# svip-lab/impersonator

Hardware: AMD Instinct MI355X
Metric: frames/sec (256x256 motion-imitation, batch=8) (higher is better)
Workload: dtype bf16x3; 1 GPU; Imitator inference 256x256 batch=8, random-init ImpersonatorGenerator + synthetic SMPL, 1 source; frames=1024, batch_per_gpu=8, image_size=256, parallelism=frame-sharded replicas x1, grid_sample_align_corners=False, lanes=2, batches_per_launch_sequence=4, frames_per_launch=32, precision=bf16x3, precision_policy=auto

## Files before the change

### impersonator_amd/csrc/heads.hip

```cpp
#include <type_traits>

#include "conv.h"

namespace lwg {
namespace {

typedef float f32x16 __attribute__((ext_vector_type(16)));
typedef __bf16 bf16x8_t __attribute__((ext_vector_type(8)));

constexpr int HS_COLS = 32;
constexpr int HS_OUT = HS_COLS - 6;
constexpr int HS_KS = 4;
constexpr int HS_NF = 7 * HS_KS;
constexpr int HS_UP = 33;

__global__ __launch_bounds__(256) void heads_pack_kernel(const float *__restrict__ wh, uint4 *__restrict__ wfrag)
{
    const int i = blockIdx.x * blockDim.x + threadIdx.x;
    if (i >= HS_NF * 2 * 64) return;
    const int lane = i & 63, plane = (i >> 6) & 1, f = i >> 7;
    const int kh = f / HS_KS, ks = f - kh * HS_KS;
    const int n = lane & 31, k8 = (lane >> 5) * 8;
    const int kw = n >> 2, o = n & 3;
    bf16x8_t out;
#pragma unroll
    for (int e = 0; e < 8; ++e) {
        const int c = ks * 16 + k8 + e;
        const float v = n < 28 ? wh[((size_t)(kh * 7 + kw) * 64 + c) * 4 + o] : 0.f;
        const __bf16 hi = (__bf16)v;
        out[e] = plane == 0 ? hi : (__bf16)(v - (float)hi);
    }
    wfrag[i] = __builtin_bit_cast(uint4, out);
}

struct HeadsGeom {
    int strips, bands, band_rows;
};

struct RowRegs {
    float4 raw[2 * HS_KS];
};

__global__ __launch_bounds__(64) void heads_bf16x3_kernel(const HeadsArgs a, const uint4 *__restrict__ wfrag,
                                                          const HeadsGeom g)
{
    __shared__ float2 s_ss[64];
    __shared__ float s_u[HS_COLS * HS_UP];
    __shared__ uint4 s_bl[HS_NF * 64];
    const int lane = threadIdx.x;
    const int strip = blockIdx.x % g.strips;
    const int band = (blockIdx.x / g.strips) % g.bands;
    const int n = blockIdx.x / (g.strips * g.bands);
    const int xs0 = strip * HS_OUT;
    const int y0 = band * g.band_rows;
    const int y1 = min(y0 + g.band_rows, a.H);
    if (y0 >= y1) return;

    s_ss[lane] = a.scale_shift[(size_t)n * 64 + lane];
    bf16x8_t bh[HS_NF];
#pragma unroll
    for (int f = 0; f < HS_NF; ++f) {
        bh[f] = __builtin_bit_cast(bf16x8_t, wfrag[(f * 2 + 0) * 64 + lane]);
        s_bl[f * 64 + lane] = wfrag[(f * 2 + 1) * 64 + lane];
    }
    __syncthreads();

    const int m = lane & 31, kh2 = lane >> 5;
    const int xp = xs0 - 3 + m;
    const bool col_ok = xp >= 0 && xp < a.W;
    const float *xin = a.x + ((size_t)n * a.H * a.W + (col_ok ? xp : 0)) * 64 + kh2 * 8;
    const size_t row_stride = (size_t)a.W * 64;

    constexpr int RING = 8;
    f32x16 acc[RING];
#pragma unroll
    for (int s = 0; s < RING; ++s)
#pragma unroll
        for (int r = 0; r < 16; ++r) acc[s][r] = 0.f;

    struct Frag { bf16x8_t hi[HS_KS], lo[HS_KS]; };
    RowRegs raw[2];
    Frag frag;
    auto load_row = [&](int r, RowRegs &dst) {
        const int rc = min(max(r, 0), a.H - 1);
        const float *p = xin + (size_t)rc * row_stride;
#pragma unroll
        for (int ks = 0; ks < HS_KS; ++ks) {
            dst.raw[2 * ks] = *reinterpret_cast<const float4 *>(p + ks * 16);
            dst.raw[2 * ks + 1] = *reinterpret_cast<const float4 *>(p + ks * 16 + 4);
        }
    };
    auto convert = [&](int r, const RowRegs &src, int ks, Frag &f) {
        const bool ok = col_ok && r >= 0 && r < a.H;
        const float4 q0 = src.raw[2 * ks], q1 = src.raw[2 * ks + 1];
        const float raw8[8] = {q0.x, q0.y, q0.z, q0.w, q1.x, q1.y, q1.z, q1.w};
        const float4 *ssp = reinterpret_cast<const float4 *>(s_ss + ks * 16 + kh2 * 8);
        bf16x8_t h, l;
#pragma unroll
        for (int e2 = 0; e2 < 4; ++e2) {
            const float4 ss2 = ssp[e2];
            const float v0 = fmaxf(fmaf(raw8[2 * e2], ss2.x, ss2.y), 0.f);
            const float v1 = fmaxf(fmaf(raw8[2 * e2 + 1], ss2.z, ss2.w), 0.f);
            const __bf16 h0 = (__bf16)v0, h1 = (__bf16)v1;
            h[2 * e2] = h0;
            h[2 * e2 + 1] = h1;
            l[2 * e2] = (__bf16)(v0 - (float)h0);
            l[2 * e2 + 1] = (__bf16)(v1 - (float)h1);
        }
        const uint4 hz = __builtin_bit_cast(uint4, h), lz = __builtin_bit_cast(uint4, l);
        f.hi[ks] = __builtin_bit_cast(bf16x8_t, ok ? hz : make_uint4(0u, 0u, 0u, 0u));
        f.lo[ks] = __builtin_bit_cast(bf16x8_t, ok ? lz : make_uint4(0u, 0u, 0u, 0u));
    };

    const size_t hw = (size_t)a.H * a.W;
    const int xl = lane & 31, half = lane >> 5;
    const int oxc = min(xs0 + min(xl, HS_OUT - 1), a.W - 1);
    const float *bgp = a.pred ? a.bg + (size_t)(a.bg_bs > 1 ? n : 0) * 3 * hw : a.x;
    struct Bg { float v[2]; };
    auto load_bg = [&](int y) {
        const size_t p = (size_t)min(max(y, 0), a.H - 1) * a.W + oxc;
        Bg b;
        b.v[0] = bgp[(size_t)(half * 2) * hw + p];
        b.v[1] = bgp[(size_t)(half ? 2 : 1) * hw + p];
        return b;
    };
    struct Out { float c0, c1, msk; };
    auto tile_to_lds = [&](const f32x16 &u) {
        const int col = lane & 31, rsel = 4 * (lane >> 5);
#pragma unroll
        for (int r = 0; r < 16; ++r) s_u[((r & 3) + 8 * (r >> 2) + rsel) * HS_UP + col] = u[r];
    };
    auto reduce_row = [&]() {
        const int xr = min(xl, HS_OUT - 1);
        float s0 = 0.f, s1 = 0.f;
#pragma unroll
        for (int kw = 0; kw < 7; ++kw) {
            s0 += s_u[(xr + kw) * HS_UP + kw * 4 + half * 2];
            s1 += s_u[(xr + kw) * HS_UP + kw * 4 + half * 2 + 1];
        }
        const float e0 = __expf(2.f * s0);
        const float e1 = __expf(half ? -s1 : 2.f * s1);
        const float r0 = __builtin_amdgcn_rcpf(1.f + e0), r1 = __builtin_amdgcn_rcpf(1.f + e1);
        Out o;
        o.c0 = fmaf(-2.f, r0, 1.f);
        o.c1 = half ? r1 : fmaf(-2.f, r1, 1.f);
        o.msk = __shfl(o.c1, 32 + xl);
        return o;
    };
    auto store_row = [&](const Out &o, const Bg &b, int y) {
        const int ox = xs0 + xl;
        if (y < y0 || y >= y1 || xl >= HS_OUT || ox >= a.W) return;
        const size_t p = (size_t)y * a.W + ox;
        const float cv[2] = {o.c0, o.c1};
#pragma unroll
        for (int k = 0; k < 2; ++k) {
            const int c = half * 2 + k;
            if (c == 3) {
                if (a.mask) a.mask[(size_t)n * hw + p] = o.msk;
                continue;
            }
            if (a.color) a.color[((size_t)n * 3 + c) * hw + p] = cv[k];
            if (a.pred) a.pred[((size_t)n * 3 + c) * hw + p] = o.msk * b.v[k] + (1.f - o.msk) * cv[k];
        }
    };

    const int niter = y1 - y0 + 6;
    load_row(y0 - 3, raw[0]);
    load_row(y0 - 2, raw[1]);
#pragma unroll
    for (int ks = 0; ks < HS_KS; ++ks) convert(y0 - 3, raw[0], ks, frag);

    auto row_step = [&](int it, auto ph_c) {
        constexpr int PH = decltype(ph_c)::value;
        constexpr int PREV = (PH + RING - 1) % RING;
        const int r = y0 - 3 + it;
        const Bg bgv = load_bg(r - 4);
        load_row(r + 2, raw[PH & 1]);
        tile_to_lds(acc[PREV]);
#pragma unroll
        for (int q = 0; q < 16; ++q) acc[PREV][q] = 0.f;
        Out o;
#pragma unroll
        for (int ks = 0; ks < HS_KS; ++ks) {
            bf16x8_t bl[7];
#pragma unroll
            for (int kh = 0; kh < 7; ++kh) bl[kh] = __builtin_bit_cast(bf16x8_t, s_bl[(kh * HS_KS + ks) * 64 + lane]);
#pragma unroll
            for (int t = 0; t < 3; ++t)
#pragma unroll
                for (int kh = 0; kh < 7; ++kh) {
                    const int slot = (PH - kh + 6 + RING) % RING;
                    const bf16x8_t av = t == 0 ? frag.lo[ks] : frag.hi[ks];
                    const bf16x8_t bv = t == 2 ? bl[kh] : bh[kh * HS_KS + ks];
                    acc[slot] = __builtin_amdgcn_mfma_f32_32x32x16_bf16(av, bv, acc[slot], 0, 0, 0);
                }
            if (ks == 1) o = reduce_row();
            convert(r + 1, raw[(PH + 1) & 1], ks, frag);
#pragma unroll
            for (int g2 = 0; g2 < 21; ++g2) {
                __builtin_amdgcn_sched_group_barrier(0x008, 1, 0);
                __builtin_amdgcn_sched_group_barrier(0x002, 6, 0);
                __builtin_amdgcn_sched_group_barrier(0x100, 1, 0);
            }
            __builtin_amdgcn_sched_barrier(0);
        }
        store_row(o, bgv, r - 4);
    };

    for (int it = 0; it < niter; it += RING) {
        row_step(it, std::integral_constant<int, 0>{});
        if (it + 1 < niter) row_step(it + 1, std::integral_constant<int, 1>{});
        if (it + 2 < niter) row_step(it + 2, std::integral_constant<int, 2>{});
        if (it + 3 < niter) row_step(it + 3, std::integral_constant<int, 3>{});
        if (it + 4 < niter) row_step(it + 4, std::integral_constant<int, 4>{});
        if (it + 5 < niter) row_step(it + 5, std::integral_constant<int, 5>{});
        if (it + 6 < niter) row_step(it + 6, std::integral_constant<int, 6>{});
        if (it + 7 < niter) row_step(it + 7, std::integral_constant<int, 7>{});
    }
    {
        const int last = niter - 1, y = y0 - 3 + last - 3;
        const Bg bgv = load_bg(y);
        switch (last % RING) {
            case 0: tile_to_lds(acc[0]); break;
            case 1: tile_to_lds(acc[1]); break;
            case 2: tile_to_lds(acc[2]); break;
            case 3: tile_to_lds(acc[3]); break;
            case 4: tile_to_lds(acc[4]); break;
            case 5: tile_to_lds(acc[5]); break;
            case 6: tile_to_lds(acc[6]); break;
            default: tile_to_lds(acc[7]); break;
        }
        const Out o = reduce_row();
        store_row(o, bgv, y);
    }
}

}

size_t heads_bf16x3_frag_bytes() { return (size_t)HS_NF * 2 * 64 * 16; }

int launch_heads_pack(const float *wh, void *wfrag, hipStream_t st)
{
    heads_pack_kernel<<<ceil_div(HS_NF * 2 * 64, 256), 256, 0, st>>>(wh, static_cast<uint4 *>(wfrag));
    LWG_LAUNCH_CHECK("heads_pack_kernel");
    return LWG_OK;
}

int launch_heads_bf16x3(const HeadsArgs &a, const void *wfrag, hipStream_t st, int bands_forced)
{
    if (a.pred && !a.bg) LWG_FAIL(LWG_ERR_INVALID_ARG, "heads: pred requested without a background image");
    if (!wfrag) LWG_FAIL(LWG_ERR_STATE, "heads: packed weight fragments missing");
    if (a.N < 1 || a.H < 1 || a.W < 1 || bands_forced < 0) LWG_FAIL(LWG_ERR_INVALID_ARG, "heads: empty tensor or negative band count");
    HeadsGeom g;
    g.strips = ceil_div(a.W, HS_OUT);
    const int target = 4 * device_cu_count();
    int bands = target / (g.strips * a.N);
    if (bands < 1) bands = 1;
    if (bands > ceil_div(a.H, 8)) bands = ceil_div(a.H, 8);
    if (bands_forced > 0) bands = bands_forced < a.H ? bands_forced : a.H;
    g.band_rows = ceil_div(a.H, bands);
    g.bands = ceil_div(a.H, g.band_rows);
    heads_bf16x3_kernel<<<g.strips * g.bands * a.N, 64, 0, st>>>(a, static_cast<const uint4 *>(wfrag), g);
    LWG_LAUNCH_CHECK("heads_bf16x3_kernel");
    return LWG_OK;
}

}
```

Measured before the change: 3931 frames/s.

## Hand-interleave heads conv MFMA loop with loads, conversion, reduction; add trace probe

Restructures the heads kernel's inner row step so each of the 21 MFMAs per k-slice is paired with a slice of other work: LDS weight loads, split bf16 hi/lo conversion, staged tile-to-LDS writes, reduction reads and activation, all fenced with scheduling barriers and register pins. The aim is to hide LDS latency and VALU work behind the matrix instructions instead of relying on the sched_group_barrier hints. It also adds an optional timing-trace variant behind a compile flag and an environment variable. The manual schedule increases register pressure and makes the code fragile.

```diff
diff --git a/impersonator_amd/csrc/heads.hip b/impersonator_amd/csrc/heads.hip
--- a/impersonator_amd/csrc/heads.hip
+++ b/impersonator_amd/csrc/heads.hip
@@ -1,3 +1,5 @@
+#include <cstdio>
+#include <cstdlib>
 #include <type_traits>
 
 #include "conv.h"
@@ -7,6 +9,9 @@
 
 typedef float f32x16 __attribute__((ext_vector_type(16)));
 typedef __bf16 bf16x8_t __attribute__((ext_vector_type(8)));
+typedef __bf16 bf16x2_t __attribute__((ext_vector_type(2)));
+typedef unsigned u32x4 __attribute__((ext_vector_type(4)));
+typedef float f32x4 __attribute__((ext_vector_type(4)));
 
 constexpr int HS_COLS = 32;
 constexpr int HS_OUT = HS_COLS - 6;
@@ -41,9 +46,29 @@
     float4 raw[2 * HS_KS];
 };
 
-__global__ __launch_bounds__(64) void heads_bf16x3_kernel(const HeadsArgs a, const uint4 *__restrict__ wfrag,
-                                                          const HeadsGeom g)
-{
+template <bool TRACE>
+__device__ __forceinline__ void heads_bf16x3_body(const HeadsArgs &a, const uint4 *__restrict__ wfrag, const HeadsGeom &g,
+                                                  unsigned long long *__restrict__ trace)
+{
+    auto stamp = [&]() -> unsigned long long {
+        if constexpr (TRACE) {
+            __builtin_amdgcn_sched_barrier(0);
+            const unsigned long long t = __builtin_amdgcn_s_memtime();
+            __builtin_amdgcn_sched_barrier(0);
+            return t;
+        }
+        return 0ull;
+    };
+    unsigned long long tr_vm = 0, tr_lgkm = 0, tr_cal = 0, tr_ks[HS_KS] = {0, 0, 0, 0}, tr_store = 0;
+    const unsigned long long tr_in = stamp();
+    unsigned long long tr_rt0 = 0;
+    if constexpr (TRACE) {
+        tr_rt0 = __builtin_amdgcn_s_memrealtime();
+        const unsigned long long c0 = stamp();
+        asm volatile("s_waitcnt lgkmcnt(0)" ::: "memory");
+        const unsigned long long c1 = stamp();
+        tr_cal = c1 - c0;
+    }
     __shared__ float2 s_ss[64];
     __shared__ float s_u[HS_COLS * HS_UP];
     __shared__ uint4 s_bl[HS_NF * 64];
@@ -55,6 +80,7 @@
     const int y0 = band * g.band_rows;
     const int y1 = min(y0 + g.band_rows, a.H);
     if (y0 >= y1) return;
+    const int tr_stores = (a.color ? 2 : 0) + (a.mask ? 1 : 0) + (a.pred ? 2 : 0);
 
     s_ss[lane] = a.scale_shift[(size_t)n * 64 + lane];
     bf16x8_t bh[HS_NF];
@@ -81,14 +107,15 @@
     struct Frag { bf16x8_t hi[HS_KS], lo[HS_KS]; };
     RowRegs raw[2];
     Frag frag;
-    auto load_row = [&](int r, RowRegs &dst) {
+    auto load_row_part = [&](int r, RowRegs &dst, int ks) {
         const int rc = min(max(r, 0), a.H - 1);
         const float *p = xin + (size_t)rc * row_stride;
-#pragma unroll
-        for (int ks = 0; ks < HS_KS; ++ks) {
-            dst.raw[2 * ks] = *reinterpret_cast<const float4 *>(p + ks * 16);
-            dst.raw[2 * ks + 1] = *reinterpret_cast<const float4 *>(p + ks * 16 + 4);
-        }
+        dst.raw[2 * ks] = *reinterpret_cast<const float4 *>(p + ks * 16);
+        dst.raw[2 * ks + 1] = *reinterpret_cast<const float4 *>(p + ks * 16 + 4);
+    };
+    auto load_row = [&](int r, RowRegs &dst) {
+#pragma unroll
+        for (int ks = 0; ks < HS_KS; ++ks) load_row_part(r, dst, ks);
     };
     auto convert = [&](int r, const RowRegs &src, int ks, Frag &f) {
         const bool ok = col_ok && r >= 0 && r < a.H;
@@ -110,6 +137,12 @@
         const uint4 hz = __builtin_bit_cast(uint4, h), lz = __builtin_bit_cast(uint4, l);
         f.hi[ks] = __builtin_bit_cast(bf16x8_t, ok ? hz : make_uint4(0u, 0u, 0u, 0u));
         f.lo[ks] = __builtin_bit_cast(bf16x8_t, ok ? lz : make_uint4(0u, 0u, 0u, 0u));
+    };
+
+    auto pin = [](bf16x8_t &v) {
+        u32x4 t = __builtin_bit_cast(u32x4, v);
+        asm volatile("" : "+v"(t));
+        v = __builtin_bit_cast(bf16x8_t, t);
     };
 
     const size_t hw = (size_t)a.H * a.W;
@@ -125,19 +158,20 @@
         return b;
     };
     struct Out { float c0, c1, msk; };
-    auto tile_to_lds = [&](const f32x16 &u) {
+    auto tile_to_lds = [&](f32x16 &u, int q) {
         const int col = lane & 31, rsel = 4 * (lane >> 5);
 #pragma unroll
-        for (int r = 0; r < 16; ++r) s_u[((r & 3) + 8 * (r >> 2) + rsel) * HS_UP + col] = u[r];
-    };
-    auto reduce_row = [&]() {
-        const int xr = min(xl, HS_OUT - 1);
-        float s0 = 0.f, s1 = 0.f;
-#pragma unroll
-        for (int kw = 0; kw < 7; ++kw) {
-            s0 += s_u[(xr + kw) * HS_UP + kw * 4 + half * 2];
-            s1 += s_u[(xr + kw) * HS_UP + kw * 4 + half * 2 + 1];
-        }
+        for (int r = 4 * q; r < 4 * q + 4; ++r) {
+            s_u[((r & 3) + 8 * (r >> 2) + rsel) * HS_UP + col] = u[r];
+            u[r] = 0.f;
+        }
+    };
+    const int xr = min(xl, HS_OUT - 1);
+    auto reduce_read = [&](int kw, float &u0, float &u1) {
+        u0 = s_u[(xr + kw) * HS_UP + kw * 4 + half * 2];
+        u1 = s_u[(xr + kw) * HS_UP + kw * 4 + half * 2 + 1];
+    };
+    auto activate = [&](float s0, float s1) {
         const float e0 = __expf(2.f * s0);
         const float e1 = __expf(half ? -s1 : 2.f * s1);
         const float r0 = __builtin_amdgcn_rcpf(1.f + e0), r1 = __builtin_amdgcn_rcpf(1.f + e1);
@@ -170,43 +204,120 @@
 #pragma unroll
     for (int ks = 0; ks < HS_KS; ++ks) convert(y0 - 3, raw[0], ks, frag);
 
+    f32x4 ssv[4];
+#pragma unroll
+    for (int q = 0; q < 4; ++q) ssv[q] = reinterpret_cast<const f32x4 *>(s_ss + kh2 * 8)[q];
+
     auto row_step = [&](int it, auto ph_c) {
         constexpr int PH = decltype(ph_c)::value;
         constexpr int PREV = (PH + RING - 1) % RING;
         const int r = y0 - 3 + it;
-        const Bg bgv = load_bg(r - 4);
-        load_row(r + 2, raw[PH & 1]);
-        tile_to_lds(acc[PREV]);
-#pragma unroll
-        for (int q = 0; q < 16; ++q) acc[PREV][q] = 0.f;
+        const bool ok = col_ok && r + 1 >= 0 && r + 1 < a.H;
+        const RowRegs &src = raw[(PH + 1) & 1];
+        Bg bgv;
         Out o;
+        float s0 = 0.f, s1 = 0.f, u0[7], u1[7];
+        unsigned long long tk[HS_KS + 1];
 #pragma unroll
         for (int ks = 0; ks < HS_KS; ++ks) {
-            bf16x8_t bl[7];
-#pragma unroll
-            for (int kh = 0; kh < 7; ++kh) bl[kh] = __builtin_bit_cast(bf16x8_t, s_bl[(kh * HS_KS + ks) * 64 + lane]);
-#pragma unroll
-            for (int t = 0; t < 3; ++t)
-#pragma unroll
-                for (int kh = 0; kh < 7; ++kh) {
-                    const int slot = (PH - kh + 6 + RING) % RING;
-                    const bf16x8_t av = t == 0 ? frag.lo[ks] : frag.hi[ks];
-                    const bf16x8_t bv = t == 2 ? bl[kh] : bh[kh * HS_KS + ks];
-                    acc[slot] = __builtin_amdgcn_mfma_f32_32x32x16_bf16(av, bv, acc[slot], 0, 0, 0);
-                }
-            if (ks == 1) o = reduce_row();
-            convert(r + 1, raw[(PH + 1) & 1], ks, frag);
-#pragma unroll
-            for (int g2 = 0; g2 < 21; ++g2) {
-                __builtin_amdgcn_sched_group_barrier(0x008, 1, 0);
-                __builtin_amdgcn_sched_group_barrier(0x002, 6, 0);
-                __builtin_amdgcn_sched_group_barrier(0x100, 1, 0);
+            tk[ks] = stamp();
+            u32x4 bl[7];
+            const float4 q0 = src.raw[2 * ks], q1 = src.raw[2 * ks + 1];
+            const float raw8[8] = {q0.x, q0.y, q0.z, q0.w, q1.x, q1.y, q1.z, q1.w};
+            float v0 = 0.f, v1 = 0.f;
+            unsigned h[4], l[4];
+#pragma unroll
+            for (int j = 0; j < 21; ++j) {
+                const int t = j / 7, kh = j - 7 * t;
+                const int slot = (PH - kh + 6 + RING) % RING;
+                if constexpr (TRACE) {
+                    if (j == 14) {
+                        const unsigned long long t0 = stamp();
+                        asm volatile("s_waitcnt lgkmcnt(0)" ::: "memory");
+                        const unsigned long long t1 = stamp();
+                        tr_lgkm += t1 - t0;
+                    }
+                }
+                const bf16x8_t av = t == 0 ? frag.lo[ks] : frag.hi[ks];
+                const bf16x8_t bv = t == 2 ? __builtin_bit_cast(bf16x8_t, bl[kh]) : bh[kh * HS_KS + ks];
+                acc[slot] = __builtin_amdgcn_mfma_f32_32x32x16_bf16(av, bv, acc[slot], 0, 0, 0);
+                if (j < 7) bl[j] = *reinterpret_cast<const u32x4 *>(&s_bl[(j * HS_KS + ks) * 64 + lane]);
+                if (j == 13) {
+#pragma unroll
+                    for (int q = 0; q < 7; ++q) asm volatile("" : "+v"(bl[q]));
+                    const f32x4 *ssp = reinterpret_cast<const f32x4 *>(s_ss + ((ks + 1) % HS_KS) * 16 + kh2 * 8);
+#pragma unroll
+                    for (int q = 0; q < 4; ++q) ssv[q] = ssp[q];
+                }
+                if (j == 20) {
+#pragma unroll
+                    for (int q = 0; q < 4; ++q) asm volatile("" : "+v"(ssv[q]));
+                }
+                if (ks == 0 && j == 13) bgv = load_bg(r - 4);
+                if (ks == 0 && j >= 14 && j <= 17) load_row_part(r + 2, raw[PH & 1], j - 14);
+                if (ks == 0 && j == 17) {
+                    if constexpr (TRACE) {
+                        const int younger = (r - 5 >= y0 && r - 5 < y1 ? tr_stores : 0);
+                        const unsigned long long t0 = stamp();
+                        switch (younger) {
+                            case 0: asm volatile("s_waitcnt vmcnt(10)" ::: "memory"); break;
+                            case 1: asm volatile("s_waitcnt vmcnt(11)" ::: "memory"); break;
+                            case 2: asm volatile("s_waitcnt vmcnt(12)" ::: "memory"); break;
+                            case 3: asm volatile("s_waitcnt vmcnt(13)" ::: "memory"); break;
+                            case 4: asm volatile("s_waitcnt vmcnt(14)" ::: "memory"); break;
+                            default: asm volatile("s_waitcnt vmcnt(15)" ::: "memory"); break;
+                        }
+                        const unsigned long long t1 = stamp();
+                        tr_vm += t1 - t0;
+                    }
+                }
+                if (ks == 0 && j >= 1 && j <= 4) tile_to_lds(acc[PREV], j - 1);
+                if (j >= 5 && j <= 12) {
+                    const int e2 = (j - 5) >> 1;
+                    if (((j - 5) & 1) == 0) {
+                        v0 = fmaxf(fmaf(raw8[2 * e2], ssv[e2][0], ssv[e2][1]), 0.f);
+                        v1 = fmaxf(fmaf(raw8[2 * e2 + 1], ssv[e2][2], ssv[e2][3]), 0.f);
+                        const bf16x2_t h2 = {(__bf16)v0, (__bf16)v1};
+                        h[e2] = __builtin_bit_cast(unsigned, h2);
+                        asm volatile("" : "+v"(v0), "+v"(v1), "+v"(h[e2]));
+                    } else {
+                        const bf16x2_t h2 = __builtin_bit_cast(bf16x2_t, h[e2]);
+                        const bf16x2_t l2 = {(__bf16)(v0 - (float)h2[0]), (__bf16)(v1 - (float)h2[1])};
+                        l[e2] = ok ? __builtin_bit_cast(unsigned, l2) : 0u;
+                        h[e2] = ok ? h[e2] : 0u;
+                        asm volatile("" : "+v"(l[e2]), "+v"(h[e2]));
+                    }
+                }
+                if (ks == 1 && j < 7) reduce_read(j, u0[j], u1[j]);
+                if (ks == 1 && j == 13) {
+#pragma unroll
+                    for (int kw = 0; kw < 7; ++kw) asm volatile("" : "+v"(u0[kw]), "+v"(u1[kw]));
+                }
+                if (ks == 1 && j >= 14) {
+                    s0 += u0[j - 14];
+                    s1 += u1[j - 14];
+                }
+                if (ks == 2 && j == 13) {
+                    o = activate(s0, s1);
+                    asm volatile("" : "+v"(o.c0), "+v"(o.c1), "+v"(o.msk));
+                }
+                __builtin_amdgcn_sched_barrier(0);
             }
-            __builtin_amdgcn_sched_barrier(0);
-        }
+            const u32x4 hv = {h[0], h[1], h[2], h[3]}, lv = {l[0], l[1], l[2], l[3]};
+            frag.hi[ks] = __builtin_bit_cast(bf16x8_t, hv);
+            frag.lo[ks] = __builtin_bit_cast(bf16x8_t, lv);
+        }
+        tk[HS_KS] = stamp();
         store_row(o, bgv, r - 4);
-    };
-
+        if constexpr (TRACE) {
+            const unsigned long long te = stamp();
+#pragma unroll
+            for (int ks = 0; ks < HS_KS; ++ks) tr_ks[ks] += tk[ks + 1] - tk[ks];
+            tr_store += te - tk[HS_KS];
+        }
+    };
+
+    const unsigned long long tr_loop0 = stamp();
     for (int it = 0; it < niter; it += RING) {
         row_step(it, std::integral_constant<int, 0>{});
         if (it + 1 < niter) row_step(it + 1, std::integral_constant<int, 1>{});
@@ -217,23 +328,108 @@
         if (it + 6 < niter) row_step(it + 6, std::integral_constant<int, 6>{});
         if (it + 7 < niter) row_step(it + 7, std::integral_constant<int, 7>{});
     }
+    const unsigned long long tr_loop1 = stamp();
     {
         const int last = niter - 1, y = y0 - 3 + last - 3;
         const Bg bgv = load_bg(y);
+        auto whole_tile = [&](f32x16 &u) {
+#pragma unroll
+            for (int q = 0; q < 4; ++q) tile_to_lds(u, q);
+        };
         switch (last % RING) {
-            case 0: tile_to_lds(acc[0]); break;
-            case 1: tile_to_lds(acc[1]); break;
-            case 2: tile_to_lds(acc[2]); break;
-            case 3: tile_to_lds(acc[3]); break;
-            case 4: tile_to_lds(acc[4]); break;
-            case 5: tile_to_lds(acc[5]); break;
-            case 6: tile_to_lds(acc[6]); break;
-            default: tile_to_lds(acc[7]); break;
-        }
-        const Out o = reduce_row();
+            case 0: whole_tile(acc[0]); break;
+            case 1: whole_tile(acc[1]); break;
+            case 2: whole_tile(acc[2]); break;
+            case 3: whole_tile(acc[3]); break;
+            case 4: whole_tile(acc[4]); break;
+            case 5: whole_tile(acc[5]); break;
+            case 6: whole_tile(acc[6]); break;
+            default: whole_tile(acc[7]); break;
+        }
+        float s0 = 0.f, s1 = 0.f;
+#pragma unroll
+        for (int kw = 0; kw < 7; ++kw) {
+            float u0, u1;
+            reduce_read(kw, u0, u1);
+            s0 += u0;
+            s1 += u1;
+        }
+        const Out o = activate(s0, s1);
         store_row(o, bgv, y);
     }
-}
+    if constexpr (TRACE) {
+        asm volatile("s_waitcnt vmcnt(0)" ::: "memory");
+        const unsigned long long tr_end = stamp(), rt1 = __builtin_amdgcn_s_memrealtime();
+        if (lane == 0) {
+            unsigned long long *rec = trace + (size_t)blockIdx.x * 16;
+            rec[0] = tr_end - tr_in;
+            rec[1] = tr_loop0 - tr_in;
+            rec[2] = tr_loop1 - tr_loop0;
+            rec[3] = tr_vm;
+            rec[4] = tr_lgkm;
+            rec[5] = tr_end - tr_loop1;
+            rec[6] = (unsigned long long)niter;
+            rec[7] = tr_cal;
+            rec[8] = rt1 - tr_rt0;
+            rec[9] = tr_rt0;
+            for (int ks = 0; ks < HS_KS; ++ks) rec[10 + ks] = tr_ks[ks];
+            rec[14] = tr_store;
+        }
+    }
+}
+
+__global__ __launch_bounds__(64) void heads_bf16x3_kernel(const HeadsArgs a, const uint4 *__restrict__ wfrag,
+                                                          const HeadsGeom g)
+{
+    heads_bf16x3_body<false>(a, wfrag, g, nullptr);
+}
+
+#ifdef LWG_EXPERIMENTS
+__global__ __launch_bounds__(64) void heads_bf16x3_trace_kernel(const HeadsArgs a, const uint4 *__restrict__ wfrag,
+                                                                const HeadsGeom g, unsigned long long *__restrict__ trace)
+{
+    heads_bf16x3_body<true>(a, wfrag, g, trace);
+}
+
+int heads_trace_launch(const HeadsArgs &a, const uint4 *wfrag, const HeadsGeom &g, int groups, int waves_per_group,
+                       hipStream_t st, const char *path)
+{
+    const int waves = groups * waves_per_group;
+    unsigned long long *dev = nullptr;
+    LWG_HIP(hipMalloc(&dev, (size_t)waves * 16 * sizeof(unsigned long long)));
+    LWG_HIP(hipMemsetAsync(dev, 0, (size_t)waves * 16 * sizeof(unsigned long long), st));
+    heads_bf16x3_trace_kernel<<<groups, 64 * waves_per_group, 0, st>>>(a, wfrag, g, dev);
+    LWG_LAUNCH_CHECK("heads_bf16x3_trace_kernel");
+    LWG_HIP(hipStreamSynchronize(st));
+    unsigned long long *rec = static_cast<unsigned long long *>(malloc((size_t)waves * 16 * sizeof(unsigned long long)));
+    if (!rec) LWG_FAIL(LWG_ERR_STATE, "heads trace: out of host memory");
+    LWG_HIP(hipMemcpy(rec, dev, (size_t)waves * 16 * sizeof(unsigned long long), hipMemcpyDeviceToHost));
+    LWG_HIP(hipFree(dev));
+    double sum[15] = {0};
+    unsigned long long longest = 0, first = ~0ull, last = 0;
+    int ran = 0;
+    for (int w = 0; w < waves; ++w) {
+        const unsigned long long *r = rec + (size_t)w * 16;
+        if (!r[6]) continue;
+        ++ran;
+        for (int k = 0; k < 15; ++k) sum[k] += (double)r[k];
+        if (r[0] > longest) longest = r[0];
+        if (r[9] < first) first = r[9];
+        if (r[9] + r[8] > last) last = r[9] + r[8];
+    }
+    free(rec);
+    if (FILE *f = ran ? fopen(path, "a") : nullptr) {
+        const double n = ran, steps = sum[6] / n;
+        fprintf(f, "| %dx%dx%d | %d x %d | %d | %.1f | %.0f | %.0f | %.0f | %.0f | %.0f | %.0f | %.0f | %llu | %.0f | %.0f | %.0f | %.2f | %.1f | %.0f %.0f %.0f %.0f | %.0f |\n",
+                a.N, a.H, a.W, groups, waves_per_group, g.bands, steps, sum[0] / n, sum[1] / n, sum[2] / n, sum[2] / n / steps,
+                sum[3] / n, sum[4] / n, sum[5] / n, longest, sum[3] / n / steps, sum[4] / n / steps, sum[7] / n,
+                sum[0] / (sum[8] * 10.0), (double)(last - first) / 100.0, sum[10] / n / steps, sum[11] / n / steps,
+                sum[12] / n / steps, sum[13] / n / steps, sum[14] / n / steps);
+        fclose(f);
+    }
+    return LWG_OK;
+}
+#endif
 
 }
 
@@ -260,6 +456,10 @@
     if (bands_forced > 0) bands = bands_forced < a.H ? bands_forced : a.H;
     g.band_rows = ceil_div(a.H, bands);
     g.bands = ceil_div(a.H, g.band_rows);
+#ifdef LWG_EXPERIMENTS
+    if (const char *path = getenv("LWG_HEADS_TRACE"))
+        return heads_trace_launch(a, static_cast<const uint4 *>(wfrag), g, g.strips * g.bands * a.N, 1, st, path);
+#endif
     heads_bf16x3_kernel<<<g.strips * g.bands * a.N, 64, 0, st>>>(a, static_cast<const uint4 *>(wfrag), g);
     LWG_LAUNCH_CHECK("heads_bf16x3_kernel");
     return LWG_OK;
```

New measurement: 3927 frames/s. Within noise of the previous version (-0.1%).
